# preiter93/ndrustfft

Hardware: AMD Instinct MI355X
Metric: GFFT-points/s, batched 1-D C2C FFT f64 along the contiguous axis (+ achieved HBM GB/s vs roofline) (higher is better)
Workload: dtype f64

## Files before the change

### ndrustfft_amd/csrc/pow2_config.h

```cpp
#pragma once
#include "pow2_kernel.h"

namespace ndfft {

#define NDFFT_POW2_CONFIGS_F64(X) \
    X(64, 8, 8, 8)            \
    X(128, 8, 16, 8)          \
    X(256, 16, 16, 16)        \
    X(512, 64, 8, 8, 8)       \
    X(1024, 64, 16, 8, 8)     \
    X(2048, 128, 16, 16, 8)   \
    X(4096, 512, 8, 8, 8, 8)  \
    X(8192, 512, 8, 8, 8, 16) \
    X(16384, 1024, 16, 16, 16, 4)
#define NDFFT_POW2_CONFIGS_F32(X) \
    X(64, 8, 8, 8)            \
    X(128, 8, 8, 2, 8)        \
    X(256, 16, 8, 4, 8)       \
    X(512, 32, 8, 8, 8)       \
    X(1024, 64, 8, 16, 8)     \
    X(2048, 128, 8, 4, 8, 8)  \
    X(4096, 256, 8, 8, 8, 8)  \
    X(8192, 512, 8, 16, 8, 8) \
    X(16384, 512, 16, 16, 8, 8)

#ifndef NDFFT_POW2_ROW_THREADS
#define NDFFT_POW2_ROW_THREADS 256
#endif
static constexpr int lpb_for(int tpl) { return tpl >= NDFFT_POW2_ROW_THREADS ? 1 : NDFFT_POW2_ROW_THREADS / tpl; }

template <typename T, int N> struct Pow2Cfg;
#define NDFFT_DEF_CFG64(N_, TPL_, ...) \
    template <> struct Pow2Cfg<double, N_> { static constexpr int TPL = TPL_; using RL = RadixList<__VA_ARGS__>; };
#define NDFFT_DEF_CFG32(N_, TPL_, ...) \
    template <> struct Pow2Cfg<float, N_> { static constexpr int TPL = TPL_; using RL = RadixList<__VA_ARGS__>; };
NDFFT_POW2_CONFIGS_F64(NDFFT_DEF_CFG64)
NDFFT_POW2_CONFIGS_F32(NDFFT_DEF_CFG32)

template <typename T, int N> struct Pow2Half { static constexpr bool value = true; };
template <> struct Pow2Half<float, 2048> { static constexpr bool value = false; };
template <> struct Pow2Half<float, 4096> { static constexpr bool value = false; };
template <> struct Pow2Half<float, 8192> { static constexpr bool value = false; };
template <> struct Pow2Half<float, 16384> { static constexpr bool value = false; };

template <typename T, int N> struct Pow2PSplit { static constexpr int value = (sizeof(T) == 4 && N >= 8192) ? 2 : 1; };

template <typename T> constexpr int pow2_row_flags(int n, bool fused) {
    int f = fused ? 8 : 0;
    if (n >= 4096) f |= 16;
    if (n == 4096 && !fused) f |= 32 | 64;
    return f;
}
template <typename T, int N, int NT, int VEC = 1, bool FUSED = false, int PS = 1>
using Pow2RowKernel = Pow2Kernel<T, N, Pow2Cfg<T, N>::TPL, lpb_for(Pow2Cfg<T, N>::TPL), Pow2Half<T, N>::value, typename Pow2Cfg<T, N>::RL,
                                 pow2_row_flags<T>(N, FUSED), 1, NT, VEC, PS>;

template <int N> constexpr bool f32_can_vec2() {
    using RL = typename Pow2Cfg<float, N>::RL;
    constexpr int E = N / Pow2Cfg<float, N>::TPL;
    return (E / RL::at(0)) % 2 == 0 && (E / RL::at(RL::NP - 1)) % 2 == 0;
}

}
```

### ndrustfft_amd/csrc/pow2_kernel.h

```cpp
#pragma once
#include "butterflies.h"
#ifndef __HIPCC_RTC__
#include "engine.h"
#include <cmath>
#endif

namespace ndfft {

template <int... Rs> struct RadixList {
    static constexpr int NP = sizeof...(Rs);
    static constexpr int at(int i) { constexpr int r[NP] = {Rs...}; return r[i]; }
    static constexpr int ns(int i) { int s = 1; for (int p = 0; p < i; ++p) s *= at(p); return s; }
    static constexpr int twoff(int i) { int o = 0; for (int p = 1; p < i; ++p) o += (at(p) - 1) * ns(p); return o; }
};

#ifndef NDFFT_PHI_SHIFT
#define NDFFT_PHI_SHIFT 4
#endif
__device__ __forceinline__ int phi(int p) { return p + (p >> NDFFT_PHI_SHIFT); }
template <int STRIDE> __device__ __forceinline__ int phi_at(int base, int pbase, int r) {
    if constexpr (STRIDE % (1 << NDFFT_PHI_SHIFT) == 0) return pbase + r * (STRIDE + (STRIDE >> NDFFT_PHI_SHIFT));
    else return phi(base + r * STRIDE);
}
template <int Ns> __device__ __forceinline__ int kmod(int j) {
    if constexpr ((Ns & (Ns - 1)) == 0) return j & (Ns - 1);
    else return j % Ns;
}

template <typename T> struct vec_of;
template <> struct vec_of<float> { typedef float type __attribute__((ext_vector_type(2))); };
template <> struct vec_of<double> { typedef double type __attribute__((ext_vector_type(2))); };
template <typename T, bool NT> __device__ __forceinline__ cpx<T> gload(const cpx<T> *p) {
    if constexpr (NT) {
        typename vec_of<T>::type v = __builtin_nontemporal_load((const typename vec_of<T>::type *)p);
        return mk<T>(v.x, v.y);
    } else {
        return *p;
    }
}
typedef float vec4f __attribute__((ext_vector_type(4)));
template <bool NT> __device__ __forceinline__ vec4f gload4(const float *p) {
    if constexpr (NT) return __builtin_nontemporal_load((const vec4f *)p);
    else return *(const vec4f *)p;
}
template <bool NT> __device__ __forceinline__ void gstore4(float *p, vec4f v) {
    if constexpr (NT) __builtin_nontemporal_store(v, (vec4f *)p);
    else *(vec4f *)p = v;
}
template <typename T, bool NT> __device__ __forceinline__ void gstore(cpx<T> *p, cpx<T> v) {
    if constexpr (NT) {
        typename vec_of<T>::type w; w.x = v.x; w.y = v.y;
        __builtin_nontemporal_store(w, (typename vec_of<T>::type *)p);
    } else {
        *p = v;
    }
}

template <typename T> __device__ __forceinline__ cpx<T> tw_load(const cpx<T> *p) {
#if defined(__HIP_DEVICE_COMPILE__) && !defined(__HIPCC_RTC__) && !defined(NDFFT_LDS_BARRIER_OVERRIDE)
    const double *d = (const double *)p;
    if constexpr (sizeof(T) == 8) {
        return mk<T>(__hip_atomic_load(d, __ATOMIC_RELAXED, __HIP_MEMORY_SCOPE_WAVEFRONT), __hip_atomic_load(d + 1, __ATOMIC_RELAXED, __HIP_MEMORY_SCOPE_WAVEFRONT));
    } else {
        const double b = __hip_atomic_load(d, __ATOMIC_RELAXED, __HIP_MEMORY_SCOPE_WAVEFRONT);
        cpx<T> r; __builtin_memcpy(&r, &b, sizeof(r)); return r;
    }
#else
    return *p;
#endif
}
template <bool RAW> __device__ __forceinline__ void xbar() {
#ifdef NDFFT_LDS_BARRIER_OVERRIDE
    if constexpr (RAW) NDFFT_LDS_BARRIER_OVERRIDE();
#else
    if constexpr (RAW) asm volatile("s_waitcnt lgkmcnt(0)\n\ts_barrier" ::: "memory");
#endif
    else __syncthreads();
}
template <typename T, int N, int TPL, int LPB, bool HALF, typename RL, int FLAGS = 0, int MINW = 1, int NT = 1, int VEC = 1, int PSPLIT = 1> struct Pow2Kernel {
    static constexpr bool PREF = (FLAGS & 32) != 0;
    static constexpr bool DERIVE = (FLAGS & 64) != 0;
    static_assert(!DERIVE || PREF, "FLAGS bit 6 is a variant of the latency form (bit 5)");
    static constexpr bool derived(int p) { return DERIVE && (RL::at(p) == 8 || RL::at(p) == 16); }
    static constexpr int MIN_WAVES = MINW;
    static constexpr int nbfly(int p) { return N / RL::at(p); }
    static constexpr int slots(int p) { return (nbfly(p) + TPL - 1) / TPL; }
    static constexpr bool full(int p) { return nbfly(p) % TPL == 0; }
    static constexpr int calc_e() { int e = 0; for (int p = 0; p < RL::NP; ++p) { const int x = slots(p) * RL::at(p); if (x > e) e = x; } return e; }
    static constexpr int E = calc_e();
    static constexpr int THREADS = TPL * LPB;
    static_assert(PSPLIT == 1 || PSPLIT == 2, "PSPLIT is 1 or 2");
    static constexpr int LANE_LDS = N / PSPLIT + ((N / PSPLIT) >> NDFFT_PHI_SHIFT) + 1;
    static constexpr size_t LDS_BYTES = (size_t)LPB * LANE_LDS * (HALF ? sizeof(T) : 2 * sizeof(T));

    template <int P> static __device__ __forceinline__ int jof(int t, int q) {
        if constexpr (VEC == 2 && (P == 0 || P == RL::NP - 1)) return 2 * t + (q & 1) + (q >> 1) * (2 * TPL);
        else return t + q * TPL;
    }

    template <int P> static __device__ __forceinline__ void load_tw(cpx<T> (&w)[E], const cpx<T> *__restrict__ twp, int t) {
        constexpr int R = RL::at(P), Ns = RL::ns(P), NBF = slots(P), NB = nbfly(P);
        const cpx<T> *tw = twp + RL::twoff(P);
#pragma unroll
        for (int q = 0; q < NBF; ++q) {
            const int j = jof<P>(t, q), k = kmod<Ns>(j);
            if (full(P) || j < NB) {
                if constexpr (derived(P)) {
#pragma unroll
                    for (int r = 1; r < R; r *= 2) w[q * R + r] = tw_load<T>(tw + (r - 1) * Ns + k);
                } else {
#pragma unroll
                    for (int r = 1; r < R; ++r) w[q * R + r] = tw[(r - 1) * Ns + k];
                }
            }
        }
    }
    template <int P>
    static __device__ __forceinline__ void passes(cpx<T> (&v)[E], const cpx<T> *__restrict__ twp, char *lds, int t) {
        if constexpr (PREF) { cpx<T> w[E]; passes_w<P>(v, twp, lds, t, w); }
        else { cpx<T> w[1]; passes_w<P>(v, twp, lds, t, w); }
    }
    template <int P, int WN>
    static __device__ __forceinline__ void passes_w(cpx<T> (&v)[E], const cpx<T> *__restrict__ twp, char *lds, int t, cpx<T> (&wpre)[WN]) {
        constexpr int R = RL::at(P), Ns = RL::ns(P), NBF = slots(P), NB = nbfly(P);
        constexpr bool FULL = full(P);
        constexpr bool TW_POWERS = (FLAGS & 16) != 0 && (size_t)(R - 1) * Ns * sizeof(cpx<T>) > 32 * 1024;
        static_assert(!PREF || !TW_POWERS || DERIVE, "the latency form loads plain tables (bit 5 alone) or the power rows of every radix-8 / 16 pass (bits 5 + 6)");
        if constexpr (P > 0 && !(FLAGS & 1) && PREF) {
#pragma unroll
            for (int q = 0; q < NBF; ++q) {
                if (FULL || jof<P>(t, q) < NB) {
                    if constexpr (derived(P)) {
                        cpx<T> *w = &wpre[q * R];
                        w[3] = cmul(w[1], w[2]); w[5] = cmul(w[1], w[4]); w[6] = cmul(w[2], w[4]); w[7] = cmul(w[3], w[4]);
                        if constexpr (R == 16) {
#pragma unroll
                            for (int r = 9; r < 16; ++r) w[r] = cmul(w[r - 8], w[8]);
                        }
                    }
#pragma unroll
                    for (int r = 1; r < R; ++r) v[q * R + r] = cmul(v[q * R + r], wpre[q * R + r]);
                }
            }
            if constexpr (DERIVE && P + 1 < RL::NP) load_tw<P + 1>(wpre, twp, t);
        } else
        if constexpr (P > 0 && !(FLAGS & 1)) {
            const cpx<T> *tw = twp + RL::twoff(P);
#pragma unroll
            for (int q = 0; q < NBF; ++q) {
                const int j = jof<P>(t, q), k = kmod<Ns>(j);
                if (FULL || j < NB) {
                    if constexpr (TW_POWERS && (R == 8 || R == 16)) {
                        cpx<T> w[R];
                        w[1] = tw[k]; w[2] = tw[Ns + k]; w[4] = tw[3 * Ns + k];
                        w[3] = cmul(w[1], w[2]); w[5] = cmul(w[1], w[4]); w[6] = cmul(w[2], w[4]); w[7] = cmul(w[3], w[4]);
                        if constexpr (R == 16) {
                            w[8] = tw[7 * Ns + k];
#pragma unroll
                            for (int r = 9; r < 16; ++r) w[r] = cmul(w[r - 8], w[8]);
                        }
#pragma unroll
                        for (int r = 1; r < R; ++r) v[q * R + r] = cmul(v[q * R + r], w[r]);
                    } else {
#pragma unroll
                        for (int r = 1; r < R; ++r) v[q * R + r] = cmul(v[q * R + r], tw[(r - 1) * Ns + k]);
                    }
                }
            }
        }
#pragma unroll
        for (int q = 0; q < NBF; ++q) if constexpr (!(FLAGS & 4)) { if (FULL || jof<P>(t, q) < NB) Bfly<T, R>::run(&v[q * R]); }
        if constexpr (P + 1 < RL::NP) {
            constexpr int R2 = RL::at(P + 1), NB2 = N / R2, NBF2 = slots(P + 1);
            constexpr bool FULL2 = full(P + 1);
            if constexpr (PREF && !DERIVE && !(FLAGS & 1)) load_tw<P + 1>(wpre, twp, t);
            if constexpr (FLAGS & 2) {
            } else if constexpr (HALF) {
                T *s = (T *)lds;
#pragma unroll
                for (int half = 0; half < 2; ++half) {
                    T keep[PSPLIT == 2 ? NBF2 * (R2 / 2) : 1];
#pragma unroll
                    for (int ps = 0; ps < PSPLIT; ++ps) {
                        xbar<PREF>();
#pragma unroll
                        for (int q = 0; q < NBF; ++q) {
                            const int j = jof<P>(t, q), k = kmod<Ns>(j), o = (j - k) * R + k - ps * (N / 2), po = phi(o);
                            if ((FULL || j < NB) && (PSPLIT == 1 || (j < NB / 2) == (ps == 0))) {
#pragma unroll
                                for (int r = 0; r < R; ++r) s[phi_at<Ns>(o, po, r)] = half ? v[q * R + r].y : v[q * R + r].x;
                            }
                        }
                        xbar<PREF>();
#pragma unroll
                        for (int q = 0; q < NBF2; ++q) {
                            const int j = jof<P + 1>(t, q), pj = phi(j);
                            if (FULL2 || j < NB2) {
#pragma unroll
                                for (int r = 0; r < R2 / PSPLIT; ++r) {
                                    const T x = s[phi_at<NB2>(j, pj, r)];
                                    if constexpr (PSPLIT == 2) {
                                        if (ps == 0) { keep[q * (R2 / 2) + r] = x; continue; }
                                    }
                                    const int rr = r + ps * (R2 / 2);
                                    if (half) v[q * R2 + rr].y = x; else v[q * R2 + rr].x = x;
                                }
                            }
                        }
                    }
                    if constexpr (PSPLIT == 2) {
#pragma unroll
                        for (int q = 0; q < NBF2; ++q)
#pragma unroll
                            for (int r = 0; r < R2 / 2; ++r) { if (half) v[q * R2 + r].y = keep[q * (R2 / 2) + r]; else v[q * R2 + r].x = keep[q * (R2 / 2) + r]; }
                    }
                }
            } else {
                cpx<T> *s = (cpx<T> *)lds;
                cpx<T> keep[PSPLIT == 2 ? NBF2 * (R2 / 2) : 1];
#pragma unroll
                for (int ps = 0; ps < PSPLIT; ++ps) {
                    xbar<PREF>();
#pragma unroll
                    for (int q = 0; q < NBF; ++q) {
                        const int j = jof<P>(t, q), k = kmod<Ns>(j), o = (j - k) * R + k - ps * (N / 2), po = phi(o);
                        if ((FULL || j < NB) && (PSPLIT == 1 || (j < NB / 2) == (ps == 0))) {
#pragma unroll
                            for (int r = 0; r < R; ++r) s[phi_at<Ns>(o, po, r)] = v[q * R + r];
                        }
                    }
                    xbar<PREF>();
#pragma unroll
                    for (int q = 0; q < NBF2; ++q) {
                        const int j = jof<P + 1>(t, q), pj = phi(j);
                        if (FULL2 || j < NB2) {
#pragma unroll
                            for (int r = 0; r < R2 / PSPLIT; ++r) {
                                const cpx<T> x = s[phi_at<NB2>(j, pj, r)];
                                if constexpr (PSPLIT == 2) {
                                    if (ps == 0) { keep[q * (R2 / 2) + r] = x; continue; }
                                }
                                v[q * R2 + r + ps * (R2 / 2)] = x;
                            }
                        }
                    }
                }
                if constexpr (PSPLIT == 2) {
#pragma unroll
                    for (int q = 0; q < NBF2; ++q)
#pragma unroll
                        for (int r = 0; r < R2 / 2; ++r) v[q * R2 + r] = keep[q * (R2 / 2) + r];
                }
            }
            passes_w<P + 1>(v, twp, lds, t, wpre);
        }
    }

    static __device__ __forceinline__ void run(const Pow2Args &a) {
        extern __shared__ __attribute__((aligned(16))) char smem[];
        const int t = threadIdx.x % TPL, ll = threadIdx.x / TPL;
        const int64_t lane = (int64_t)xcd_block(blockIdx.x, gridDim.x, a.xcd_chunk) * LPB + ll;
        const bool live = lane < a.nlanes;
        const cpx<T> *in = (const cpx<T> *)a.in + (live ? lane : 0) * a.pitch_in;
        cpx<T> *out = (cpx<T> *)a.out + (live ? lane : 0) * a.pitch_out;
        char *lds = smem + (size_t)ll * LANE_LDS * (HALF ? sizeof(T) : 2 * sizeof(T));
        cpx<T> v[E];
        {
            constexpr int R0 = RL::at(0), NB0 = N / R0, NBF0 = slots(0);
            if constexpr (VEC == 2) {
                static_assert(NBF0 % 2 == 0 && full(0) && full(RL::NP - 1), "VEC=2 needs an even number of whole butterfly rounds in the first and last pass");
#pragma unroll
                for (int q = 0; q < NBF0; q += 2)
#pragma unroll
                    for (int r = 0; r < R0; ++r) {
                        const vec4f w = gload4<(NT & 2) != 0>((const float *)(in + jof<0>(t, q) + r * NB0));
                        v[q * R0 + r] = mk<T>(w.x, w.y); v[(q + 1) * R0 + r] = mk<T>(w.z, w.w);
                    }
            } else {
#pragma unroll
                for (int q = 0; q < NBF0; ++q)
                    if (full(0) || t + q * TPL < NB0) {
#pragma unroll
                        for (int r = 0; r < R0; ++r) v[q * R0 + r] = gload<T, (NT & 2) != 0>(in + t + q * TPL + r * NB0);
                    }
            }
        }
        cpx<T> w[DERIVE ? E : 1];
        if constexpr (DERIVE && RL::NP > 1 && !(FLAGS & 1)) load_tw<1>(w, (const cpx<T> *)a.twp, t);
        if (a.inverse) {
#pragma unroll
            for (int i = 0; i < E; ++i) v[i].y = -v[i].y;
        }
        if constexpr ((FLAGS & 8) != 0) {
            constexpr int R0 = RL::at(0), NB0 = N / R0, NBF0 = slots(0);
            const int k1 = (int)(lane % a.f1), mask = (1 << a.logB) - 1;
            const cpx<T> *lo = (const cpx<T> *)a.twlo, *hi = (const cpx<T> *)a.twhi;
#pragma unroll
            for (int q = 0; q < NBF0; ++q)
                if (full(0) || jof<0>(t, q) < NB0) {
#pragma unroll
                    for (int r = 0; r < R0; ++r) {
                        const int m = (jof<0>(t, q) + r * NB0) * k1;
                        v[q * R0 + r] = cmul(v[q * R0 + r], cmul(hi[m >> a.logB], lo[m & mask]));
                    }
                }
        }
        if constexpr (DERIVE) passes_w<0>(v, (const cpx<T> *)a.twp, lds, t, w);
        else passes<0>(v, (const cpx<T> *)a.twp, lds, t);
        if (!live) return;
        constexpr int RL_ = RL::at(RL::NP - 1), NBL = N / RL_, NBFL = slots(RL::NP - 1);
        if (a.inverse) {
            const T sc = (T)a.scale;
#pragma unroll
            for (int i = 0; i < E; ++i) { v[i].x *= sc; v[i].y *= -sc; }
        }
        if constexpr (VEC == 2) {
            static_assert(NBFL % 2 == 0, "VEC=2 needs an even number of butterflies per thread in the last pass");
#pragma unroll
            for (int q = 0; q < NBFL; q += 2)
#pragma unroll
                for (int r = 0; r < RL_; ++r) {
                    vec4f w; w.x = v[q * RL_ + r].x; w.y = v[q * RL_ + r].y; w.z = v[(q + 1) * RL_ + r].x; w.w = v[(q + 1) * RL_ + r].y;
                    gstore4<(NT & 1) != 0>((float *)(out + jof<RL::NP - 1>(t, q) + r * NBL), w);
                }
        } else {
#pragma unroll
            for (int q = 0; q < NBFL; ++q)
                if (full(RL::NP - 1) || t + q * TPL < NBL) {
#pragma unroll
                    for (int r = 0; r < RL_; ++r) gstore<T, (NT & 1) != 0>(out + t + q * TPL + r * NBL, v[q * RL_ + r]);
                }
        }
    }
};

template <typename K> __global__ __launch_bounds__(K::THREADS, K::MIN_WAVES) void k_pow2(const Pow2Args a) { K::run(a); }

#ifndef __HIPCC_RTC__
template <typename RL> inline void build_tw(HostTable &out) {
    const long double kPiL = 3.14159265358979323846264338327950288L;
    for (int p = 1; p < RL::NP; ++p) {
        const int R = RL::at(p), Ns = RL::ns(p);
        for (int r = 1; r < R; ++r)
            for (int k = 0; k < Ns; ++k) {
                const unsigned long long num = ((unsigned long long)r * k) % ((unsigned long long)Ns * R);
                const long double ang = 2.0L * kPiL * (long double)num / (long double)((unsigned long long)Ns * R);
                out.re.push_back(cosl(ang)); out.im.push_back(-sinl(ang));
            }
    }
}


#endif

}
```

Baseline: 184.8.

## Make first f64 4096-point exchange wave-private to drop block barriers

For the f64 4096-point unfused row kernel (radix 8.8.8.8 on 512 threads), threads are permuted so the data exchanged after pass 0 stays inside one wavefront. That exchange then uses a custom LDS slot layout and a plain lgkmcnt wait in place of the workgroup s_barrier. The aim is to remove block-wide barrier stalls between the first two passes. In exchange it adds a permuted thread-to-element mapping for the global loads, a larger padded LDS footprint, and a correctness risk if the layout or the wave-level sync assumptions are wrong.

```diff
diff --git a/ndrustfft_amd/csrc/pow2_config.h b/ndrustfft_amd/csrc/pow2_config.h
--- a/ndrustfft_amd/csrc/pow2_config.h
+++ b/ndrustfft_amd/csrc/pow2_config.h
@@ -49,6 +49,7 @@
     int f = fused ? 8 : 0;
     if (n >= 4096) f |= 16;
     if (n == 4096 && !fused) f |= 32 | 64;
+    if (n == 4096 && !fused && sizeof(T) == 8) f |= 128;
     return f;
 }
 template <typename T, int N, int NT, int VEC = 1, bool FUSED = false, int PS = 1>
diff --git a/ndrustfft_amd/csrc/pow2_kernel.h b/ndrustfft_amd/csrc/pow2_kernel.h
--- a/ndrustfft_amd/csrc/pow2_kernel.h
+++ b/ndrustfft_amd/csrc/pow2_kernel.h
@@ -22,6 +22,13 @@
     if constexpr (STRIDE % (1 << NDFFT_PHI_SHIFT) == 0) return pbase + r * (STRIDE + (STRIDE >> NDFFT_PHI_SHIFT));
     else return phi(base + r * STRIDE);
 }
+constexpr int WL_LDS = 8 * 584;
+constexpr int wl_perm(int t) { return (t & 7) | (((t >> 6) & 7) << 3) | (((t >> 3) & 7) << 6); }
+template <int P> constexpr int wl_slot(int p) {
+    if constexpr (P == 0) return 584 * (p >> 9) + 72 * ((p >> 6) & 7) + 36 * ((p >> 5) & 1) + ((p >> 3) & 3) + 4 * (p & 7);
+    else return 584 * (p >> 9) + 72 * ((p >> 3) & 7) + 8 * ((p >> 6) & 7) + (p & 7);
+}
+template <int P, int STRIDE> constexpr int wl_at(int pbase, int r) { return pbase + r * (wl_slot<P>(STRIDE) - wl_slot<P>(0)); }
 template <int Ns> __device__ __forceinline__ int kmod(int j) {
     if constexpr ((Ns & (Ns - 1)) == 0) return j & (Ns - 1);
     else return j % Ns;
@@ -77,10 +84,21 @@
 #endif
     else __syncthreads();
 }
+__device__ __forceinline__ void wave_lds_sync() {
+#ifdef NDFFT_LDS_BARRIER_OVERRIDE
+    NDFFT_LDS_BARRIER_OVERRIDE();
+#else
+    asm volatile("s_waitcnt lgkmcnt(0)" ::: "memory");
+#endif
+}
 template <typename T, int N, int TPL, int LPB, bool HALF, typename RL, int FLAGS = 0, int MINW = 1, int NT = 1, int VEC = 1, int PSPLIT = 1> struct Pow2Kernel {
     static constexpr bool PREF = (FLAGS & 32) != 0;
     static constexpr bool DERIVE = (FLAGS & 64) != 0;
     static_assert(!DERIVE || PREF, "FLAGS bit 6 is a variant of the latency form (bit 5)");
+    static constexpr bool WL1 = (FLAGS & 128) != 0, WL3 = (FLAGS & 256) != 0, WL = WL1 || WL3;
+    static constexpr bool wl_radices() { for (int p = 0; p < RL::NP; ++p) if (RL::at(p) != 8) return false; return RL::NP == 4; }
+    static_assert(!WL || (N == 4096 && TPL == 512 && LPB == 1 && HALF && VEC == 1 && PSPLIT == 1 && wl_radices()), "FLAGS bits 7 and 8 are written for 4096 = 8.8.8.8 on 512 threads, half exchange");
+    static constexpr bool wave_private(int p) { return (WL1 && p == 0) || (WL3 && p == 2); }
     static constexpr bool derived(int p) { return DERIVE && (RL::at(p) == 8 || RL::at(p) == 16); }
     static constexpr int MIN_WAVES = MINW;
     static constexpr int nbfly(int p) { return N / RL::at(p); }
@@ -90,11 +108,13 @@
     static constexpr int E = calc_e();
     static constexpr int THREADS = TPL * LPB;
     static_assert(PSPLIT == 1 || PSPLIT == 2, "PSPLIT is 1 or 2");
-    static constexpr int LANE_LDS = N / PSPLIT + ((N / PSPLIT) >> NDFFT_PHI_SHIFT) + 1;
+    static constexpr int PHI_LDS = N / PSPLIT + ((N / PSPLIT) >> NDFFT_PHI_SHIFT) + 1;
+    static constexpr int LANE_LDS = WL && WL_LDS > PHI_LDS ? WL_LDS : PHI_LDS;
     static constexpr size_t LDS_BYTES = (size_t)LPB * LANE_LDS * (HALF ? sizeof(T) : 2 * sizeof(T));
 
     template <int P> static __device__ __forceinline__ int jof(int t, int q) {
         if constexpr (VEC == 2 && (P == 0 || P == RL::NP - 1)) return 2 * t + (q & 1) + (q >> 1) * (2 * TPL);
+        else if constexpr ((WL1 && P == 0) || (WL3 && P >= 2)) return wl_perm(t);
         else return t + q * TPL;
     }
 
@@ -172,7 +192,7 @@
         for (int q = 0; q < NBF; ++q) if constexpr (!(FLAGS & 4)) { if (FULL || jof<P>(t, q) < NB) Bfly<T, R>::run(&v[q * R]); }
         if constexpr (P + 1 < RL::NP) {
             constexpr int R2 = RL::at(P + 1), NB2 = N / R2, NBF2 = slots(P + 1);
-            constexpr bool FULL2 = full(P + 1);
+            constexpr bool FULL2 = full(P + 1), PRIV = wave_private(P);
             if constexpr (PREF && !DERIVE && !(FLAGS & 1)) load_tw<P + 1>(wpre, twp, t);
             if constexpr (FLAGS & 2) {
             } else if constexpr (HALF) {
@@ -182,23 +202,25 @@
                     T keep[PSPLIT == 2 ? NBF2 * (R2 / 2) : 1];
 #pragma unroll
                     for (int ps = 0; ps < PSPLIT; ++ps) {
-                        xbar<PREF>();
+                        if constexpr (!PRIV) xbar<PREF>();
+                        else if (P > 0 && half == 0) xbar<PREF>();
+                        else if (half) wave_lds_sync();
 #pragma unroll
                         for (int q = 0; q < NBF; ++q) {
-                            const int j = jof<P>(t, q), k = kmod<Ns>(j), o = (j - k) * R + k - ps * (N / 2), po = phi(o);
+                            const int j = jof<P>(t, q), k = kmod<Ns>(j), o = (j - k) * R + k - ps * (N / 2), po = PRIV ? wl_slot<P>(o) : phi(o);
                             if ((FULL || j < NB) && (PSPLIT == 1 || (j < NB / 2) == (ps == 0))) {
 #pragma unroll
-                                for (int r = 0; r < R; ++r) s[phi_at<Ns>(o, po, r)] = half ? v[q * R + r].y : v[q * R + r].x;
+                                for (int r = 0; r < R; ++r) s[PRIV ? wl_at<P, Ns>(po, r) : phi_at<Ns>(o, po, r)] = half ? v[q * R + r].y : v[q * R + r].x;
                             }
                         }
-                        xbar<PREF>();
+                        if constexpr (PRIV) wave_lds_sync(); else xbar<PREF>();
 #pragma unroll
                         for (int q = 0; q < NBF2; ++q) {
-                            const int j = jof<P + 1>(t, q), pj = phi(j);
+                            const int j = jof<P + 1>(t, q), pj = PRIV ? wl_slot<P>(j) : phi(j);
                             if (FULL2 || j < NB2) {
 #pragma unroll
                                 for (int r = 0; r < R2 / PSPLIT; ++r) {
-                                    const T x = s[phi_at<NB2>(j, pj, r)];
+                                    const T x = s[PRIV ? wl_at<P, NB2>(pj, r) : phi_at<NB2>(j, pj, r)];
                                     if constexpr (PSPLIT == 2) {
                                         if (ps == 0) { keep[q * (R2 / 2) + r] = x; continue; }
                                     }
@@ -265,6 +287,7 @@
         cpx<T> *out = (cpx<T> *)a.out + (live ? lane : 0) * a.pitch_out;
         char *lds = smem + (size_t)ll * LANE_LDS * (HALF ? sizeof(T) : 2 * sizeof(T));
         cpx<T> v[E];
+        const int t0 = jof<0>(t, 0), tl = jof<RL::NP - 1>(t, 0);
         {
             constexpr int R0 = RL::at(0), NB0 = N / R0, NBF0 = slots(0);
             if constexpr (VEC == 2) {
@@ -279,9 +302,9 @@
             } else {
 #pragma unroll
                 for (int q = 0; q < NBF0; ++q)
-                    if (full(0) || t + q * TPL < NB0) {
-#pragma unroll
-                        for (int r = 0; r < R0; ++r) v[q * R0 + r] = gload<T, (NT & 2) != 0>(in + t + q * TPL + r * NB0);
+                    if (full(0) || t0 + q * TPL < NB0) {
+#pragma unroll
+                        for (int r = 0; r < R0; ++r) v[q * R0 + r] = gload<T, (NT & 2) != 0>(in + t0 + q * TPL + r * NB0);
                     }
             }
         }
@@ -326,9 +349,9 @@
         } else {
 #pragma unroll
             for (int q = 0; q < NBFL; ++q)
-                if (full(RL::NP - 1) || t + q * TPL < NBL) {
-#pragma unroll
-                    for (int r = 0; r < RL_; ++r) gstore<T, (NT & 1) != 0>(out + t + q * TPL + r * NBL, v[q * RL_ + r]);
+                if (full(RL::NP - 1) || tl + q * TPL < NBL) {
+#pragma unroll
+                    for (int r = 0; r < RL_; ++r) gstore<T, (NT & 1) != 0>(out + tl + q * TPL + r * NBL, v[q * RL_ + r]);
                 }
         }
     }
```

After: 186.0, median of 6. About the same (+0.6%).
